# zha0ming1e/legged_mpc_control

Measured on AMD Instinct MI355X. Metric: QP solves/sec (Go1, horizon=10, 12 contacts); max GRF err vs exact-QP oracle, higher is better.
Workload: dtype f64; 1 GPU; go1_trot_h10_b1024; horizon=10, batch_per_gpu=1024, global_batch=1024, robot=go1, gait=trot, parallelism=dp1 (independent QP shards, no collective)

## Files before the change

legged_mpc_control_amd/build.py:

```python
from __future__ import annotations

import os
import shutil
import subprocess

PKG = os.path.dirname(os.path.abspath(__file__))
ROOT = os.path.dirname(PKG)
CSRC = os.path.join(PKG, "csrc")
LIBDIR = os.path.join(PKG, "lib")
LIB = os.path.join(LIBDIR, "liblmpc.so")
ARCH = "gfx950"
HIP_FLAGS = ["-mllvm", "-amdgpu-mfma-vgpr-form"]
KERNEL_FP = ["-ffp-contract=on", "-fno-signed-zeros"]
SCHED_FLAGS = {
    "lmpc_kernels.hip": ["-mllvm", "-amdgpu-sched-strategy=max-ilp"],
    "lmpc_dense.hip": ["-mllvm", "-amdgpu-sched-strategy=max-ilp"] + KERNEL_FP,
    "lmpc_lq.hip": ["-mllvm", "-amdgpu-sched-strategy=iterative-ilp"] + KERNEL_FP,
    "lmpc_fused.hip": ["-mllvm", "-amdgpu-sched-strategy=max-ilp"] + KERNEL_FP,
    "lmpc_gi.hip": ["-mllvm", "-amdgpu-sched-strategy=iterative-ilp"],
    "lmpc_hoqp.hip": ["-mllvm", "-amdgpu-sched-strategy=iterative-ilp"],
}

SOURCES = ["lmpc_kernels.hip", "lmpc_lq.hip", "lmpc_fused.hip", "lmpc_dense.hip", "lmpc_gi.hip", "lmpc_prep.hip", "lmpc_rollout.hip", "lmpc_hoqp.hip", "lmpc_wbc.hip", "lmpc_rbd.hip", "lmpc_sim.hip", "lmpc_contact.hip", "lmpc_stack.hip", "lmpc_est.hip", "lmpc_lowlevel.hip", "lmpc_capi.cpp",
           "hoqp_capi.cpp", "lmpc_host.cpp", "ConvexQPSolver.cpp"]
# ... 47 lines not shown
        os.path.join(ROOT, "include", "lmpc", "lmpc_rollout.h"), os.path.join(ROOT, "include", "lmpc", "lmpc_rbd.h"),
        os.path.join(ROOT, "include", "lmpc", "lmpc_sim.h"), os.path.join(ROOT, "include", "lmpc", "lmpc_stack.h"),
        os.path.join(ROOT, "include", "lmpc", "lmpc_est.h"), os.path.join(ROOT, "include", "lmpc", "lmpc_contact.h"),
        os.path.join(ROOT, "include", "lmpc", "lmpc_lowlevel.h"),
        os.path.join(ROOT, "include", "lmpc", "ConvexQPSolver.hpp"),
        os.path.abspath(__file__)]
    if not force and not _stale(LIB, deps):
        return LIB
    return _compile_lib(LIB, os.path.join(LIBDIR, "obj"), verbose=verbose)


MULTI_LIB = os.path.join(LIBDIR, "liblmpc_multi.so")


def build_multi(force: bool = False, verbose: bool = False) -> str:
    src = os.path.join(CSRC, "lmpc_multi.cpp")
    deps = [src, LIB, os.path.join(ROOT, "include", "lmpc", "lmpc_multi.h"), os.path.join(ROOT, "include", "lmpc", "lmpc.h"),
            os.path.abspath(__file__)]
    if not force and not _stale(MULTI_LIB, deps):
        return MULTI_LIB
    tmp = MULTI_LIB + ".tmp"
    cmd = [hipcc(), f"--offload-arch={ARCH}", "-O2", "-fPIC", "-shared", "-std=c++17", "-I", os.path.join(ROOT, "include"), "-o", tmp, src,
           "-L", LIBDIR, "-llmpc", "-Wl,-rpath,$ORIGIN", "-L/opt/rocm/lib", "-lrccl", "-Wl,-rpath,/opt/rocm/lib"]
    if verbose:
        print(" ".join(cmd))
    subprocess.run(cmd, check=True)
    os.replace(tmp, MULTI_LIB)
    return MULTI_LIB


def build_stamps(force: bool = False) -> str:
    srcs = [os.path.join(CSRC, s) for s in SOURCES]
    out = os.path.join(ROOT, "tools", "build", "liblmpc_stamps.so")
    if not force and not _stale(out, srcs + [os.path.join(CSRC, h) for h in HEADERS]):
        return out
    return _compile_lib(out, os.path.join(ROOT, "tools", "build", "obj_stamps"), defines=["LMPC_STAMPS"])


def build_variant(tag: str, defines, force: bool = False, flags=()) -> str:
    srcs = [os.path.join(CSRC, s) for s in SOURCES]
    out = os.path.join(ROOT, "tools", "build", f"liblmpc_{tag}.so")
    if not force and not _stale(out, srcs + [os.path.join(CSRC, h) for h in HEADERS]):
        return out
    return _compile_lib(out, os.path.join(ROOT, "tools", "build", f"obj_{tag}"), defines=defines, flags=flags)


TEST_BUILD = os.path.join(ROOT, "tests", "build")
TEST_VARIANTS = {
    "bugza": (["LMPC_BUG_ZA"], ("lmpc_lq.hip", "lmpc_fused.hip")),
    "bugza_nokkt": (["LMPC_BUG_ZA", "LMPC_KKT_OFF"], ("lmpc_lq.hip", "lmpc_fused.hip")),
    "bugyaw": (["LMPC_BUG_YAW"], ("lmpc_lq.hip", "lmpc_fused.hip")),
    "bugyaw_nokkt": (["LMPC_BUG_YAW", "LMPC_KKT_OFF"], ("lmpc_lq.hip", "lmpc_fused.hip")),
    "noschur": (["LMPC_POLISH_SCHUR=0"], ("lmpc_dense.hip", "lmpc_lq.hip", "lmpc_fused.hip")),
    "diag2tile": (["LMPC_DIAG_TWO_TILES"], ("lmpc_dense.hip", "lmpc_lq.hip", "lmpc_fused.hip")),
}


def build_test_variants(force: bool = False) -> dict:
    build_native()
    out = {}
    for tag, (defines, only) in TEST_VARIANTS.items():
        path = os.path.join(TEST_BUILD, f"liblmpc_{tag}.so")
        deps = [os.path.join(CSRC, s) for s in SOURCES] + [os.path.join(CSRC, h) for h in HEADERS] + [LIB]
        if force or _stale(path, deps):
            _compile_lib(path, os.path.join(TEST_BUILD, f"obj_{tag}"), defines=defines, only=only)
        out[tag] = path
    return out


def build_cpp_test(force: bool = False) -> str:
    src = os.path.join(ROOT, "tests", "cpp", "grf_update_test.cpp")
    out = os.path.join(ROOT, "tests", "cpp", "build", "grf_update_test")
    if not force and not _stale(out, [src, LIB]):
        return out
    os.makedirs(os.path.dirname(out), exist_ok=True)
    cmd = [hipcc(), "-O2", "-std=c++17", "-I", os.path.join(ROOT, "include"), "-o", out, src,
           "-L", LIBDIR, "-llmpc", f"-Wl,-rpath,{LIBDIR}"]
    subprocess.run(cmd, check=True)
    return out


def build_cpp_multi_test(force: bool = False) -> str:
    src = os.path.join(ROOT, "tests", "cpp", "multi_test.cpp")
    out = os.path.join(ROOT, "tests", "cpp", "build", "multi_test")
    if not force and not _stale(out, [src, LIB, MULTI_LIB]):
        return out
    os.makedirs(os.path.dirname(out), exist_ok=True)
    cmd = [hipcc(), "-O2", "-std=c++17", "-I", os.path.join(ROOT, "include"), "-o", out, src,
           "-L", LIBDIR, "-llmpc_multi", "-llmpc", f"-Wl,-rpath,{LIBDIR}"]
    subprocess.run(cmd, check=True)
    return out


def build_cpp_eigen_test(force: bool = False) -> str:
    src = os.path.join(ROOT, "tests", "cpp", "eigen_dropin_test.cpp")
    stub = os.path.join(ROOT, "tests", "cpp", "eigen_dropin")
    out = os.path.join(ROOT, "tests", "cpp", "build", "eigen_dropin_test")
    hdr = os.path.join(ROOT, "include", "lmpc", "ConvexQPSolverEigen.hpp")
    if not force and not _stale(out, [src, hdr, LIB]):
        return out
    os.makedirs(os.path.dirname(out), exist_ok=True)
    cmd = [hipcc(), "-O2", "-std=c++17", "-Wall", "-I", stub, "-I", os.path.join(ROOT, "include"), "-o", out, src,
           "-L", LIBDIR, "-llmpc", f"-Wl,-rpath,{LIBDIR}"]
    subprocess.run(cmd, check=True)
    return out

# ... 94 lines not shown
```

legged_mpc_control_amd/csrc/lmpc_dense.hip:

```cpp
#include <hip/hip_runtime.h>

#include <cmath>
#include <cstdint>

#include "lmpc/lmpc.h"
#include "lmpc_device.h"
#include "lmpc_kernel_common.h"
#include "lmpc_dense_common.h"

namespace lmpc {

#ifdef LMPC_STAMPS
constexpr int DSTAMP_N = 14;
__device__ unsigned long long lmpc_dense_stamps[4096][DSTAMP_N];
#define DSTAMP_DECL unsigned long long _ds_acc[DSTAMP_N] = {}; unsigned long long _ds_t0 = __builtin_readcyclecounter();
#define DSTAMP(i) do { const unsigned long long _t = __builtin_readcyclecounter(); _ds_acc[i] += _t - _ds_t0; _ds_t0 = _t; } while (0)
#define DSTAMP_FLUSH(qp) do { if (threadIdx.x == 0 && (qp) < 4096) for (int _i = 0; _i < DSTAMP_N; ++_i) lmpc_dense_stamps[qp][_i] = _ds_acc[_i]; } while (0)
#define DS_PARAMS , unsigned long long (&_ds_acc)[DSTAMP_N], unsigned long long& _ds_t0
#define DS_ARGS , _ds_acc, _ds_t0
#else
#define DS_PARAMS
#define DS_ARGS
#define DSTAMP_DECL
#define DSTAMP(i) do {} while (0)
#define DSTAMP_FLUSH(qp) do {} while (0)
#endif

#ifdef LMPC_KKT_DIAG
__device__ double lmpc_kkt_diag_dense[LMPC_KKT_DIAG_QPS][4];
extern "C" int lmpc_debug_kkt_dense(double* out, int nqp) {
    if (nqp > LMPC_KKT_DIAG_QPS) nqp = LMPC_KKT_DIAG_QPS;
    return hipMemcpyFromSymbol(out, HIP_SYMBOL(lmpc_kkt_diag_dense), (size_t)nqp * 4 * sizeof(double)) == hipSuccess
               ? nqp : -1;
}
extern "C" int lmpc_debug_kkt_dense_clear(void) {
    static double zeros[LMPC_KKT_DIAG_QPS * 4];
    return hipMemcpyToSymbol(HIP_SYMBOL(lmpc_kkt_diag_dense), zeros, sizeof(zeros)) == hipSuccess ? 0 : -1;
}
#endif

#ifdef LMPC_REFINE_DIAG
__device__ double lmpc_refine_diag[LMPC_KKT_DIAG_QPS][4];
extern "C" int lmpc_debug_refine(double* out, int nqp) {
    if (nqp > LMPC_KKT_DIAG_QPS) nqp = LMPC_KKT_DIAG_QPS;
    return hipMemcpyFromSymbol(out, HIP_SYMBOL(lmpc_refine_diag), (size_t)nqp * 4 * sizeof(double)) == hipSuccess
               ? nqp : -1;
}
extern "C" int lmpc_debug_refine_clear(void) {
    static double zeros[LMPC_KKT_DIAG_QPS * 4];
    return hipMemcpyToSymbol(HIP_SYMBOL(lmpc_refine_diag), zeros, sizeof(zeros)) == hipSuccess ? 0 : -1;
}
#endif

}

#include "lmpc_dense_kernel.h"

namespace lmpc {

template <bool TERRAIN>
__global__ void __launch_bounds__(64) lmpc_dense_kernel(const DevParams prm, const double* __restrict__ rec,
                                                        const uint8_t* __restrict__ contact,
                                                        const double* __restrict__ normals, int batch,
                                                        double* __restrict__ grf, int32_t* __restrict__ status,
                                                        int32_t* __restrict__ iters, uint8_t* __restrict__ done_out) {
    (void)dense_body<TERRAIN>(prm, rec, contact, normals, batch, grf, status, iters, done_out);
}

template __global__ void lmpc_dense_kernel<false>(const DevParams, const double*, const uint8_t*, const double*, int,
                                                  double*, int32_t*, int32_t*, uint8_t*);
template __global__ void lmpc_dense_kernel<true>(const DevParams, const double*, const uint8_t*, const double*, int,
                                                 double*, int32_t*, int32_t*, uint8_t*);

#ifdef LMPC_STAMPS
extern "C" int lmpc_debug_condense_stamps(unsigned long long* out, int nqp) {
    if (nqp > 4096) nqp = 4096;
    return hipMemcpyFromSymbol(out, HIP_SYMBOL(lmpc_condense_stamps), (size_t)nqp * 5 * sizeof(unsigned long long)) ==
                   hipSuccess ? nqp : -1;
}
extern "C" int lmpc_debug_dense_stamps(unsigned long long* out, int nqp) {
    if (nqp > 4096) nqp = 4096;
    return hipMemcpyFromSymbol(out, HIP_SYMBOL(lmpc_dense_stamps), (size_t)nqp * DSTAMP_N * sizeof(unsigned long long)) ==
                   hipSuccess ? nqp : -1;
}
#endif

size_t dense_lds_bytes(int H) {
    const int doubles = 40 + 72 + 24 + 36 + 10 * DN_TILE + 64 * 3 + 180 + 60 + 64 + 2 * H + 12 * H + 64 + DN_SCR_MIN;
    return (size_t)doubles * sizeof(double) + (20 + 33) * sizeof(int);
}

hipError_t launch_dense(const DevParams& prm, const double* rec, const uint8_t* contact, const double* normals,
                        int batch, double* grf, int32_t* status, int32_t* iters, uint8_t* done, hipStream_t stream) {
    const size_t lds = dense_lds_bytes(prm.H);
    const dim3 grid(batch), block(LMPC_WAVE);
    if (normals) {
        (void)hipFuncSetAttribute((const void*)lmpc_dense_kernel<true>, hipFuncAttributeMaxDynamicSharedMemorySize,
                                  (int)lds);
        hipLaunchKernelGGL(lmpc_dense_kernel<true>, grid, block, lds, stream, prm, rec, contact, normals, batch, grf,
                           status, iters, done);
    } else {
        (void)hipFuncSetAttribute((const void*)lmpc_dense_kernel<false>, hipFuncAttributeMaxDynamicSharedMemorySize,
                                  (int)lds);
// ... 8 lines not shown
```

legged_mpc_control_amd/csrc/lmpc_dense_common.h:

```cpp
#pragma once
#include <hip/hip_runtime.h>

#include <cmath>
#include <cstdint>

#include "lmpc/lmpc.h"
#include "lmpc_device.h"
#include "lmpc_kernel_common.h"

namespace lmpc {

constexpr int DN_TILE = 256;
size_t dense_lds_bytes(int H);

__device__ __forceinline__ constexpr int tix(int r, int c) { return r * 4 - r * (r - 1) / 2 + (c - r); }
__device__ __forceinline__ constexpr int uix(int a, int b) { return a == 0 ? b - 1 : a == 1 ? b + 1 : 5; }
__device__ __forceinline__ int toff(int r, int c) { return (r >> 2) * 64 + (r & 3) * 16 + c; }
__device__ __forceinline__ int vidx(int b, int a) { return 16 * (b / 5) + 3 * (b % 5) + a; }
__device__ __forceinline__ int sym3(int p, int q) {
    const int lo = p < q ? p : q, hi = p < q ? q : p;
    return lo == 0 ? hi : lo == 1 ? 2 + hi : 5;
}

__device__ __forceinline__ d4 tprod(const d4& X, const d4& Y, d4 acc) {
// ... 468 lines not shown
        out.uit[i] = W[i];
        out.ui[i] = tr[(4 * i + g) * 17 + c];
    }
    return out;
}


__device__ __forceinline__ unsigned tile_masks(int nls, unsigned coupled) {
    return __builtin_amdgcn_readfirstlane(((1u << nls) - 1u) & coupled);
}
__device__ __forceinline__ int tile_mask(unsigned masks, int t) { return (int)((masks >> (5 * t)) & 31u); }

__device__ __forceinline__ double h_matvec(const DSmem& S, const ldouble* x, ldouble* tmp, int lane) {
    const int lc = lane & 15, lr = lane >> 4;
    double xr[4][4], xc[4];
#pragma unroll
    for (int b = 0; b < 4; ++b) {
#pragma unroll
        for (int i = 0; i < 4; ++i) xr[b][i] = x[16 * b + 4 * i + lr];
        xc[b] = x[16 * b + lc];
    }
    double pc[4] = {0.0, 0.0, 0.0, 0.0};
    double pr[3][4] = {{0.0, 0.0, 0.0, 0.0}, {0.0, 0.0, 0.0, 0.0}, {0.0, 0.0, 0.0, 0.0}};
#pragma unroll
    for (int r = 0; r < 4; ++r) {
#pragma unroll
        for (int c = r; c < 4; ++c) {
            const int k = tix(r, c);
#pragma unroll
            for (int i = 0; i < 4; ++i) {
                const double h = S.Ht[k * DN_TILE + i * 64 + lane];
                pc[c] = fma(h, xr[r][i], pc[c]);
                if (c > r) pr[r][i] = fma(h, xc[c], pr[r][i]);
            }
        }
    }
#pragma unroll
    for (int r = 0; r < 3; ++r) {
        double rs[4];
        row_sum4(pr[r], rs);
        if (lc == 0) {
#pragma unroll
            for (int i = 0; i < 4; ++i) tmp[16 * r + 4 * i + lr] = rs[i];
        }
    }
    double yc[4];
#pragma unroll
    for (int c = 0; c < 4; ++c) yc[c] = group_sum4(pc[c]);
    LMPC_SYNC();
    const double ys = lr == 0 ? yc[0] : lr == 1 ? yc[1] : lr == 2 ? yc[2] : yc[3];
    return ys + (lr < 3 ? tmp[lane < 48 ? lane : 0] : 0.0);
}

struct DenseRec {
    double v[4];
};
static_assert(33 + 12 * DENSE_MAX_H <= 4 * 64, "DenseRec holds a whole record");
__device__ __forceinline__ DenseRec dense_rec_load(const double* __restrict__ rec, int qp, int H, int lane) {
    const int RL = 33 + 12 * H;
    const double* rin = rec + (size_t)qp * RL;
    DenseRec r;
#pragma unroll
    for (int q = 0; q < 4; ++q) {
        const int i = lane + 64 * q;
        r.v[q] = rin[i < RL ? i : 0];
    }
    return r;
}

template <bool TERRAIN>
__device__ __forceinline__ int dense_prologue(const DevParams& prm, const DSmem& S, const DenseRec& rv,
                                              const double* __restrict__ normals, int qp, int H,
                                              unsigned long long smask, bool stl, int lane) {
    const int RL = 33 + 12 * H;
    const double dt = prm.dt;
#pragma unroll
    for (int q = 0; q < 4; ++q) {
        const int i = lane + 64 * q;
        if (i < 33) S.hdr[i] = rv.v[q];
        else if (i < RL) S.xr[i - 33] = rv.v[q];
    }
    const int rank = __builtin_amdgcn_mbcnt_hi((unsigned)(smask >> 32), __builtin_amdgcn_mbcnt_lo((unsigned)smask, 0));
    if (stl) S.lsm[rank] = lane;
    if (lane <= H) {
        const unsigned long long below = (lane >= 16) ? smask : (smask & ((1ull << (4 * lane)) - 1ull));
        S.fb[lane] = __popcll(below);
    }
    if (TERRAIN && lane < 4) {
        const double* nin = normals + (size_t)qp * 12 + 3 * lane;
        const double n0 = nin[0], n1 = nin[1], n2 = nin[2];
        const double nn = sqrt(n0 * n0 + n1 * n1 + n2 * n2);
        const double nx = n0 / nn, ny = n1 / nn, c = n2 / nn;
        const double h = 1.0 / (1.0 + c);
        const double R[9] = {1.0 - nx * nx * h, -nx * ny * h, nx, -nx * ny * h, 1.0 - ny * ny * h, ny, -nx, -ny, c};
#pragma unroll
        for (int e = 0; e < 9; ++e) S.tf[9 * lane + e] = R[e];
    }
    LMPC_SYNC();
    double iw[9];
    {
        const ldouble* R = S.hdr + LMPC_REC_ROT;
        double RI[9], Iw[9];
        for (int i = 0; i < 3; ++i)
            for (int j = 0; j < 3; ++j)
                RI[i * 3 + j] = R[i * 3 + 0] * prm.Ib[0 * 3 + j] + R[i * 3 + 1] * prm.Ib[1 * 3 + j] + R[i * 3 + 2] * prm.Ib[2 * 3 + j];
        for (int i = 0; i < 3; ++i)
// ... 69 lines not shown
```

legged_mpc_control_amd/csrc/lmpc_dense_kernel.h:

```cpp
#pragma once
#include <hip/hip_runtime.h>

#include <cmath>
#include <cstdint>

#include "lmpc/lmpc.h"
#include "lmpc_device.h"
#include "lmpc_kernel_common.h"
#include "lmpc_dense_common.h"

#ifndef DSTAMP
#define DS_PARAMS
#define DS_ARGS
#define DSTAMP_DECL
#define DSTAMP(i) do {} while (0)
#define DSTAMP_FLUSH(qp) do {} while (0)
#endif

#ifndef LMPC_POLISH_SCHUR
#define LMPC_POLISH_SCHUR 1
#endif

namespace lmpc {

constexpr int LMPC_SCHUR_KMAX = 6;
constexpr int LMPC_SCHUR_SLOPE2 = 4;
constexpr int LMPC_SCHUR_LIM2 = 10;
constexpr double LMPC_DENSE_Z0 = 1.0;
#ifdef LMPC_REFINE_DIAG
constexpr double LMPC_REFINE_SR = 0.0;
#else
constexpr double LMPC_REFINE_SR = 1e-12;
#endif

static_assert(48 + 4 * LMPC_SCHUR_KMAX + 2 * LMPC_SCHUR_KMAX + LMPC_SCHUR_KMAX * LMPC_SCHUR_KMAX <= 120 &&
                  120 + LMPC_SCHUR_KMAX + 1 <= 128, "range-space scratch layout");
constexpr int DN_SCHUR_SV = 120;

template <typename P>
__device__ __forceinline__ int ncols3(const P* T) {
    int n = 0;
#pragma unroll
    for (int q = 0; q < 3; ++q) n += (T[q] != 0.0 || T[3 + q] != 0.0 || T[6 + q] != 0.0) ? 1 : 0;
    return n;
}
__device__ __forceinline__ int wave_count3(int k) {
    return __popcll(__ballot(k & 1)) + 2 * __popcll(__ballot(k & 2)) + 4 * __popcll(__ballot(k & 4));
}
__device__ __forceinline__ int wave_prefix3(int k, unsigned long long below) {
    return __popcll(__ballot(k & 1) & below) + 2 * __popcll(__ballot(k & 2) & below) +
           4 * __popcll(__ballot(k & 4) & below);
}

struct SchurLeg {
    int kc, kr;
    bool ok;
};
__device__ __forceinline__ SchurLeg schur_leg(bool chg, int act, int bact, bool nap, const ldouble* Tb,
                                              const double Tn[9], double mu, double fzmax) {
    SchurLeg r{0, 0, true};
    if (!chg) return r;
    const bool bap = (bact & 3) == 3 || (bact & 12) == 12;
    if (bap && nap) return r;
    const int cm = act & bact;
    double Tc[9], uc[3];
    (void)leg_basis(cm, mu, fzmax, Tc, uc);
    const int nb = ncols3(Tb), nc = ncols3(Tc), nn = ncols3(Tn);
    r.kc = nc - nb;
    r.kr = nap ? nc : __popc(act & ~bact);
    r.ok = r.kc >= 0 && r.kc <= 3 && r.kr <= 3 && (!bap || !(cm & 16)) && (!nap || !((act | bact) & 16)) &&
           (nap || nn == nc - r.kr);
    return r;
}

template <bool TERRAIN>
__device__ __forceinline__ bool dense_body(const DevParams prm, const double* __restrict__ rec,
                                           const uint8_t* __restrict__ contact, const double* __restrict__ normals,
                                           int batch, double* __restrict__ grf, int32_t* __restrict__ status,
                                           int32_t* __restrict__ iters, uint8_t* __restrict__ done_out) {
    extern __shared__ __attribute__((aligned(16))) double dn_smem[];
    const int qp = blockIdx.x;
    if (qp >= batch) return true;
    const int lane = threadIdx.x;
    const int H = prm.H;
    const uint8_t cbyte = contact[(size_t)qp * 4 * H + (lane < 4 * H ? lane : 0)];
    const DenseRec rv = dense_rec_load(rec, qp, H, lane);
    const bool stl = lane < 4 * H && cbyte != 0;
    const unsigned long long smask = __ballot(stl);
    const int nls = __popcll(smask);
    if (nls > DENSE_MAX_LS || nls == 0) return false;
    const DSmem S = dcarve(dn_smem, H);
    const double mu = prm.mu, fzmax = prm.fmax, dt = prm.dt;
    DSTAMP_DECL

    const int rank = dense_prologue<TERRAIN>(prm, S, rv, normals, qp, H, smask, stl, lane);
    DSTAMP(0);
    dense_condense<TERRAIN>(prm, S, H, nls, smask, lane);
    constexpr int NT = 4;
    DSTAMP(1);

    const bool st = lane < nls;
    int lk = 0, lj = 0;
    if (st) {
        const int id = S.lsm[lane];
        lk = id >> 2;
        lj = id & 3;
    }
    double f[3], s[5], z[5], is[5];
    {
        const double cnt = st ? (double)(S.fb[lk + 1] - S.fb[lk]) : 1.0;
        f[0] = f[1] = 0.0;
        f[2] = st ? fmin(0.5 * fzmax, prm.mass * prm.grav / cnt) : 0.0;
        double o[5];
        cons_resid(f, mu, fzmax, o);
#pragma unroll
        for (int i = 0; i < 5; ++i) {
            s[i] = st ? -o[i] : 1.0;
            is[i] = 1.0 / s[i];
            z[i] = LMPC_DENSE_Z0 * is[i];
        }
    }
    double u[3] = {0.0, 0.0, 0.0}, rt[3] = {0.0, 0.0, 0.0};
    int qstatus = LMPC_QP_CONVERGED, ipm_it = 0, prounds = 0;
    bool done = false;
    enum { PRED = 0, CORR = 1, POLISH = 2 };
    const double mc = 5.0 * nls, imc = 1.0 / mc;
    double tol = prm.tol_mu;
    int att = 0, rd = 0, it_end = min(prm.max_iter, prm.dense_polish_iter), mode = PRED, act = 0;
    int keep_tiles = 0;
    unsigned cmask = 0;
    bool apex = false;
    int bact = 0;
    bool have_base = false, schur = false;
    int nsch = 0, ncol = 0;
    double mu_c = 0.0, smu = 0.0, sz = 0.0;
    d4 Tl[10], Ui[4], UiT[4];
    const int lc = lane & 15, lr = lane >> 4;
    int lblk_reg = -1, lblk_q = 0, lblk_off = 0, ldg_reg = -1;
#pragma unroll
    for (int i = 0; i < 4; ++i) {
        const int r = lr + 4 * i;
        if (r < 15 && lc < 15 && r / 3 == lc / 3) {
            lblk_reg = i;
            lblk_q = r / 3;
            lblk_off = 3 * (r % 3) + lc % 3;
            if (r == lc) ldg_reg = i;
        }
    }
#if LMPC_POLISH_SCHUR
    auto schur_ksolve = [&](const double (&cv)[LMPC_SCHUR_KMAX], double (&sv)[LMPC_SCHUR_KMAX], double& kmin) -> bool {
        constexpr int KM = LMPC_SCHUR_KMAX;
        const ldouble* U = S.scr + 48;
        const ldouble* uleg = U + 4 * KM;
        const ldouble* utyp = uleg + KM;
        const ldouble* Cb = utyp + KM;
        const ldouble* Wc = S.scr + 128;
        double Am[KM][KM], sg[KM];
        int rb_[KM];
        bool rw[KM];
#pragma unroll
        for (int i = 0; i < KM; ++i) {
            const bool iv = i < nsch;
            rw[i] = iv && utyp[iv ? i : 0] < 0.5;
            rb_[i] = iv ? (int)uleg[i] : 0;
            sg[i] = rw[i] ? -1.0 : 1.0;
        }
#pragma unroll
        for (int i = 0; i < KM; ++i) {
            const bool iv = i < nsch;
#pragma unroll
            for (int j = 0; j <= i; ++j) {
                const bool jv = j < nsch;
                double v = (iv && jv) ? Cb[KM * i + j] : (i == j ? 1.0 : 0.0);
                if (iv && jv) {
                    if (rw[i]) {
#pragma unroll
                        for (int q = 0; q < 3; ++q) v = fma(-U[4 * i + q], Wc[64 * j + vidx(rb_[i], q)], v);
                    } else if (rw[j]) {
#pragma unroll
                        for (int q = 0; q < 3; ++q) v = fma(-U[4 * j + q], Wc[64 * i + vidx(rb_[j], q)], v);
                    }
                }
                Am[i][j] = v;
            }
        }
        bool bad = false;
        double dd[KM];
#pragma unroll
        for (int c = 0; c < KM; ++c) {
            double d = Am[c][c];
#pragma unroll
            for (int b = 0; b < c; ++b) d = fma(-Am[c][b], Am[c][b] * dd[b], d);
            bad |= !(sg[c] * d > 1e-14 * fabs(Am[c][c]));
            if (c < nsch) kmin = fmin(kmin, fabs(d) / fabs(Am[c][c]));
            dd[c] = d;
            const double inv = rcp_nr(d != 0.0 ? d : 1.0);
#pragma unroll
            for (int r = c + 1; r < KM; ++r) {
                double v = Am[r][c];
#pragma unroll
                for (int b = 0; b < c; ++b) v = fma(-Am[r][b], Am[c][b] * dd[b], v);
                Am[r][c] = v * inv;
            }
        }
#pragma unroll
        for (int r = 0; r < KM; ++r) {
            double v = cv[r];
#pragma unroll
            for (int b = 0; b < r; ++b) v = fma(-Am[r][b], sv[b], v);
            sv[r] = v;
        }
#pragma unroll
        for (int r = 0; r < KM; ++r) sv[r] = sv[r] * rcp_nr(dd[r] != 0.0 ? dd[r] : 1.0);
#pragma unroll
        for (int r = KM - 1; r >= 0; --r) {
            double v = sv[r];
#pragma unroll
            for (int b = r + 1; b < KM; ++b) v = fma(-Am[b][r], sv[b], v);
            sv[r] = v;
        }
        return bad;
    };
    bool force_fact = false, refact_done = false;
#endif
    for (;;) {
        if (mode == PRED) {
            if (ipm_it >= prm.dense_iter_cap) break;
            double loc = 0.0;
            if (st) {
#pragma unroll
                for (int i = 0; i < 5; ++i) loc += s[i] * z[i];
            }
            DSTAMP(2);
            sz = wave_sum(loc);
            mu_c = sz * imc;
            DSTAMP(12);
            if (mu_c < tol || ipm_it >= it_end) {
                act = 0;
                if (st) {
#pragma unroll
                    for (int i = 0; i < 5; ++i)
                        if (z[i] > LMPC_ACT_RATIO * s[i]) act |= 1 << i;
                    const double fm = fmax(fabs(f[0]), fmax(fabs(f[1]), fabs(f[2])));
                    if (fm < 1e-6 * fzmax) act = 15;
                }
                mode = POLISH;
                rd = 0;
                keep_tiles = 0;
                have_base = false;
            } else {
                double W[5] = {0, 0, 0, 0, 0}, wv[5] = {0, 0, 0, 0, 0};
                if (st) {
#pragma unroll
                    for (int i = 0; i < 5; ++i) {
                        W[i] = z[i] * is[i];
                        wv[i] = W[i] * (s[i] - (i == 4 ? fzmax : 0.0));
                    }
                }
                const double sx = W[0] + W[1], sy = W[2] + W[3];
                if (st) {
                    ldouble* bk = S.blk + 9 * lane;
                    const double dxz = mu * (W[0] - W[1]), dyz = mu * (W[2] - W[3]), dzz = mu * mu * (sx + sy) + W[4];
                    bk[0] = sx;  bk[1] = 0.0; bk[2] = dxz;
                    bk[3] = 0.0; bk[4] = sy;  bk[5] = dyz;
                    bk[6] = dxz; bk[7] = dyz; bk[8] = dzz;
                }
                cons_tw(wv, mu, rt);
            }
            DSTAMP(13);
        }
        double Tn[9], upn[3];
        if (mode == POLISH) {
            ++prounds;
            apex = false;
            double (&T)[9] = Tn;
            if (st) apex = leg_basis(act, mu, fzmax, T, upn);
            schur = false;
#if LMPC_POLISH_SCHUR
            if (have_base && !force_fact) {
                const SchurLeg sl = schur_leg(st && act != bact, act, bact, apex, S.blk + 9 * lane, T, mu, fzmax);
                const int k = sl.kc + sl.kr;
                nsch = wave_count3(k);
                ncol = wave_count3(sl.kc);
                const unsigned long long dif = __ballot(st && act != bact);
                const int kt = dif ? (__ffsll((long long)dif) - 1) / 5 : 4;
                schur = __all(sl.ok) && nsch + ncol <= LMPC_SCHUR_KMAX &&
                        2 * nsch + LMPC_SCHUR_SLOPE2 * kt <= LMPC_SCHUR_LIM2;
            }
            if (!schur) {
                const unsigned long long dif = __ballot(have_base && act != bact);
                keep_tiles = have_base && dif ? (__ffsll((long long)dif) - 1) / 5 : 0;
                force_fact = false;
            }
#endif
        }
        if (mode == POLISH && !schur) {
            S.vec2[lane] = 0.0;
            LMPC_SYNC();
            bool coupled = false;
            if (st) {
                const double (&T)[9] = Tn;
                const double (&up)[3] = upn;
#pragma unroll
                for (int p = 0; p < 3; ++p) S.lup[3 * lane + p] = up[p];
                ldouble* bk = S.blk + 9 * lane;
#pragma unroll
                for (int e = 0; e < 9; ++e) bk[e] = T[e];
#pragma unroll
                for (int e = 0; e < 9; ++e) coupled |= T[e] != 0.0;
#pragma unroll
                for (int p = 0; p < 3; ++p) S.vec2[vidx(lane, p)] = up[p];
            }
            cmask = (unsigned)__ballot(coupled);
        }
        if (schur) {
        } else if (mode != POLISH) {
            if (st) {
#pragma unroll
                for (int a = 0; a < 3; ++a) S.vec[vidx(lane, a)] = -(S.gv[vidx(lane, a)] + rt[a]);
            }
            LMPC_SYNC();
        } else {
            LMPC_SYNC();
            const double hv = h_matvec(S, S.vec2, S.scr, lane) + S.gv[lane];
            LMPC_SYNC();
            S.vec2[lane] = hv;
#if LMPC_POLISH_SCHUR
            S.lhg[lane] = hv;
#endif
            LMPC_SYNC();
            if (st) {
#pragma unroll
                for (int a = 0; a < 3; ++a) {
                    double v = 0.0;
#pragma unroll
                    for (int p = 0; p < 3; ++p) v += S.blk[9 * lane + p * 3 + a] * S.vec2[vidx(lane, p)];
                    S.vec[vidx(lane, a)] = -v;
                }
            }
// ... 96 lines not shown
                if (b > 0) {
                    double part = 0.0;
#pragma unroll
                    for (int a = 0; a < b; ++a) {
#pragma unroll
                        for (int i = 0; i < 4; ++i) part = fma(Tl[tix(a, b)][i], y[a][i], part);
                    }
                    acc -= group_sum4(part);
                }
                double pp[4], rs[4];
#pragma unroll
                for (int i = 0; i < 4; ++i) pp[i] = UiT[b][i] * acc;
                row_sum4(pp, rs);
#pragma unroll
                for (int i = 0; i < 4; ++i) y[b][i] = rs[i];
            }
            double xcol[4];
#pragma unroll
            for (int b = 3; b >= 0; --b) {
                if (b >= NT) continue;
                d4 acc = y[b];
                if (b + 1 < NT) {
                    double part[4] = {0.0, 0.0, 0.0, 0.0};
#pragma unroll
                    for (int c = b + 1; c < 4; ++c) {
                        if (c >= NT) continue;
#pragma unroll
                        for (int i = 0; i < 4; ++i) part[i] = fma(Tl[tix(b, c)][i], xcol[c], part[i]);
                    }
                    double rs[4];
                    row_sum4(part, rs);
#pragma unroll
                    for (int i = 0; i < 4; ++i) acc[i] -= rs[i];
                }
                double p = 0.0;
#pragma unroll
                for (int i = 0; i < 4; ++i) p = fma(UiT[b][i], acc[i], p);
                xcol[b] = group_sum4(p);
            }
            if (lr == 0) {
#pragma unroll
                for (int b = 0; b < 4; ++b) {
                    if (b >= NT) continue;
                    S.vec[16 * b + lc] = xcol[b];
                }
            }
            LMPC_SYNC();
        };
        double du[3] = {0.0, 0.0, 0.0};
        if (!schur) {
            solve_vec();
#if LMPC_POLISH_SCHUR
            if (mode == POLISH) {
                S.lua[lane] = S.vec[lane];
                bact = act;
                have_base = true;
            }
#endif
        }
#if LMPC_POLISH_SCHUR
        else {
            constexpr int KM = LMPC_SCHUR_KMAX;
            ldouble* U = S.scr + 48;
            ldouble* uleg = U + 4 * KM;
            ldouble* utyp = uleg + KM;
            ldouble* Cb = utyp + KM;
            ldouble* Wc = S.scr + 128;
            ldouble* Vc = Wc + 64 * nsch;
            const SchurLeg sl = schur_leg(st && act != bact, act, bact, apex, S.blk + 9 * lane, Tn, mu, fzmax);
            const unsigned long long below = (1ull << lane) - 1ull;
            const int e0 = wave_prefix3(sl.kc + sl.kr, below), c0 = wave_prefix3(sl.kc, below);
            if (lane < KM * KM) Cb[lane] = 0.0;
            LMPC_SYNC();
            if (sl.kc + sl.kr) {
                const ldouble* Tb = S.blk + 9 * lane;
                const ldouble* ub = S.lup + 3 * lane;
                double Tc[9], uc[3];
                (void)leg_basis(act & bact, mu, fzmax, Tc, uc);
                double tv[3][3];
                const int nb = ncols3(Tb);
                if (nb == 0) {
#pragma unroll
                    for (int j = 0; j < 3; ++j)
#pragma unroll
                        for (int p = 0; p < 3; ++p) tv[j][p] = Tc[3 * p + j];
                } else {
                    double best = -1.0, rb[3] = {0.0, 0.0, 0.0};
#pragma unroll
                    for (int q = 0; q < 3; ++q) {
                        double r[3] = {Tc[q], Tc[3 + q], Tc[6 + q]};
#pragma unroll
                        for (int m = 0; m < 2; ++m) {
                            const double pr = Tb[m] * r[0] + Tb[3 + m] * r[1] + Tb[6 + m] * r[2];
#pragma unroll
                            for (int p = 0; p < 3; ++p) r[p] = fma(-pr, Tb[3 * p + m], r[p]);
                        }
                        const double n2 = r[0] * r[0] + r[1] * r[1] + r[2] * r[2];
                        if (n2 > best) {
                            best = n2;
                            rb[0] = r[0]; rb[1] = r[1]; rb[2] = r[2];
                        }
                    }
                    const double in = rsq_nr(best > 0.0 ? best : 1.0);
#pragma unroll
                    for (int p = 0; p < 3; ++p) tv[0][p] = rb[p] * in;
                    const double b0 = Tb[0], b1 = Tb[3], b2 = Tb[6];
                    tv[1][0] = b1 * tv[0][2] - b2 * tv[0][1];
                    tv[1][1] = b2 * tv[0][0] - b0 * tv[0][2];
                    tv[1][2] = b0 * tv[0][1] - b1 * tv[0][0];
                    tv[2][0] = tv[2][1] = tv[2][2] = 0.0;
                }
                double rv[3][3], rbv[3];
                if (apex) {
#pragma unroll
                    for (int j = 0; j < 3; ++j) {
#pragma unroll
                        for (int p = 0; p < 3; ++p) rv[j][p] = Tc[3 * p + j];
                        rbv[j] = 0.0;
                    }
                } else {
                    const ActiveRows ar = active_rows(act & ~bact);
                    cons_rowvec(ar.i0, mu, rv[0]);
                    cons_rowvec(ar.i1, mu, rv[1]);
                    cons_rowvec(ar.i2, mu, rv[2]);
                    rbv[0] = ar.i0 == 4 ? fzmax : 0.0;
                    rbv[1] = ar.i1 == 4 ? fzmax : 0.0;
                    rbv[2] = ar.i2 == 4 ? fzmax : 0.0;
                }
#pragma unroll
                for (int j = 0; j < 3; ++j) {
                    if (j >= sl.kc) continue;
                    const int e = e0 + j;
                    double c = 0.0;
#pragma unroll
                    for (int p = 0; p < 3; ++p) {
                        U[4 * e + p] = tv[j][p];
                        c = fma(-tv[j][p], S.lhg[vidx(lane, p)], c);
                    }
                    U[4 * e + 3] = c;
                    uleg[e] = (double)lane;
                    utyp[e] = (double)(1 + c0 + j);
                }
#pragma unroll
                for (int i = 0; i < 3; ++i) {
                    if (i >= sl.kr) continue;
                    const int e = e0 + sl.kc + i;
#pragma unroll
                    for (int q = 0; q < 3; ++q)
                        U[4 * e + q] = fma(rv[i][0], Tb[q], fma(rv[i][1], Tb[3 + q], rv[i][2] * Tb[6 + q]));
                    U[4 * e + 3] = rbv[i] - fma(rv[i][0], ub[0], fma(rv[i][1], ub[1], rv[i][2] * ub[2]));
                    uleg[e] = (double)lane;
                    utyp[e] = 0.0;
#pragma unroll
                    for (int j = 0; j < 3; ++j) {
                        if (j >= sl.kc) continue;
                        const double a = rv[i][0] * tv[j][0] + rv[i][1] * tv[j][1] + rv[i][2] * tv[j][2];
                        Cb[KM * e + e0 + j] = a;
                        Cb[KM * (e0 + j) + e] = a;
                    }
                }
            }
            LMPC_SYNC();
            if (ncol) {
                const int w16 = lane & 15, bl = 5 * (lane >> 4) + w16 / 3, al = w16 % 3;
                const bool vl = w16 < 15 && bl < nls;
                for (int e = 0; e < nsch; ++e) {
                    const double ty = utyp[e];
                    if (ty < 0.5) continue;
                    const int be = (int)uleg[e];
                    S.vec2[lane] = 0.0;
                    LMPC_SYNC();
                    if (lane < 3) S.vec2[vidx(be, lane)] = U[4 * e + lane];
                    LMPC_SYNC();
                    const double h = h_matvec(S, S.vec2, S.scr, lane);
                    LMPC_SYNC();
                    S.vec2[lane] = h;
                    LMPC_SYNC();
                    double v = 0.0;
                    if (vl) {
#pragma unroll
                        for (int p = 0; p < 3; ++p) v = fma(S.blk[9 * bl + 3 * p + al], S.vec2[vidx(bl, p)], v);
                    }
                    Vc[64 * ((int)ty - 1) + lane] = v;
                    if (lane < nsch && utyp[lane] > 0.5) {
                        const int bj = (int)uleg[lane];
                        double c = 0.0;
#pragma unroll
                        for (int p = 0; p < 3; ++p) c = fma(U[4 * lane + p], S.vec2[vidx(bj, p)], c);
                        Cb[KM * lane + e] = c;
                    }
                    LMPC_SYNC();
                }
            }
            for (int e = 0; e < nsch; ++e) {
                const double ty = utyp[e];
                if (ty > 0.5) {
                    S.vec[lane] = Vc[64 * ((int)ty - 1) + lane];
                } else {
                    S.vec[lane] = 0.0;
                    LMPC_SYNC();
                    if (lane < 3) S.vec[vidx((int)uleg[e], lane)] = U[4 * e + lane];
                }
                LMPC_SYNC();
                solve_vec();
                Wc[64 * e + lane] = S.vec[lane];
            }
            LMPC_SYNC();
            if (ncol) {
                const double y0l = S.lua[lane];
                for (int e = 0; e < nsch; ++e) {
                    const double ty = utyp[e];
                    if (ty < 0.5) continue;
                    const double vl = Vc[64 * ((int)ty - 1) + lane];
                    const double cy = wave_sum(vl * y0l);
                    if (lane == 0) U[4 * e + 3] -= cy;
                    for (int f = e; f < nsch; ++f) {
                        if (utyp[f] < 0.5) continue;
                        const double g = wave_sum(vl * Wc[64 * f + lane]);
                        if (lane == 0) {
                            Cb[KM * e + f] -= g;
                            if (f != e) Cb[KM * f + e] -= g;
                        }
                    }
                }
                LMPC_SYNC();
            }
            double cv[KM], sv[KM];
#pragma unroll
            for (int i = 0; i < KM; ++i) {
                const bool iv = i < nsch;
                const bool rwi = iv && utyp[iv ? i : 0] < 0.5;
                const int rbi = iv ? (int)uleg[i] : 0;
                double c = iv ? U[4 * i + 3] : 0.0;
                if (rwi) {
#pragma unroll
                    for (int q = 0; q < 3; ++q) c = fma(-U[4 * i + q], S.lua[vidx(rbi, q)], c);
                }
                cv[i] = c;
            }
            double kmin = 1.0;
            const bool bad = schur_ksolve(cv, sv, kmin);
            double yv = S.lua[lane];
#pragma unroll
            for (int j = 0; j < KM; ++j)
                if (j < nsch) yv = fma(-Wc[64 * j + lane], sv[j], yv);
            if (ncol && !bad && st) {
#pragma unroll
                for (int j = 0; j < KM; ++j) {
                    if (j >= nsch || utyp[j] < 0.5 || (int)uleg[j] != lane) continue;
#pragma unroll
                    for (int p = 0; p < 3; ++p) du[p] = fma(U[4 * j + p], sv[j], du[p]);
                }
            }
            if (lane == 0) {
#pragma unroll
                for (int j = 0; j < KM; ++j) S.scr[DN_SCHUR_SV + j] = sv[j];
                S.scr[DN_SCHUR_SV + KM] = kmin;
            }
            S.vec[lane] = bad ? S.lua[lane] : yv;
            if (bad) have_base = false;
            LMPC_SYNC();
        }
#endif
        DSTAMP(5);
        u[0] = u[1] = u[2] = 0.0;
        if (st) {
            double y3[3];
#pragma unroll
            for (int a = 0; a < 3; ++a) y3[a] = S.vec[vidx(lane, a)];
            if (mode == POLISH) {
                const ldouble* Tb = S.blk + 9 * lane;
#pragma unroll
                for (int p = 0; p < 3; ++p)
                    u[p] = apex ? 0.0
                                : S.lup[3 * lane + p] + Tb[p * 3] * y3[0] + Tb[p * 3 + 1] * y3[1] + Tb[p * 3 + 2] * y3[2] +
                                      du[p];
            } else {
#pragma unroll
                for (int p = 0; p < 3; ++p) u[p] = y3[p];
            }
        }
        if (mode == PRED) {
            double amax = 1.0;
            double dsa[5], dza[5];
#pragma unroll
            for (int i = 0; i < 5; ++i) dsa[i] = dza[i] = 0.0;
            if (st) {
#pragma unroll
                for (int m = 0; m < 3; ++m) S.lua[3 * lane + m] = u[m];
            }
            if (st) {
                double o[5];
                cons_resid(u, mu, fzmax, o);
#pragma unroll
                for (int i = 0; i < 5; ++i) {
                    dsa[i] = -o[i] - s[i];
                    dza[i] = -z[i] - z[i] * is[i] * dsa[i];
                    if (dsa[i] < 0.0) amax = fmin(amax, -s[i] * __builtin_amdgcn_rcp(dsa[i]));
                    if (dza[i] < 0.0) amax = fmin(amax, -z[i] * __builtin_amdgcn_rcp(dza[i]));
                }
            }
            const double aa = wave_min(amax);
            double loc = 0.0;
            if (st) {
#pragma unroll
                for (int i = 0; i < 5; ++i) loc += (s[i] + aa * dsa[i]) * (z[i] + aa * dza[i]);
            }
            const double ratio = wave_sum(loc) / sz;
            smu = ratio * ratio * ratio * mu_c;
            if (st) {
                double wv[5];
#pragma unroll
                for (int i = 0; i < 5; ++i)
                    wv[i] = (z[i] * (s[i] - (i == 4 ? fzmax : 0.0)) + smu - dsa[i] * dza[i]) * is[i];
// ... 214 lines not shown
#pragma unroll
                            for (int i = 0; i < 5; ++i)
                                if (!((act >> i) & 1) && o[i] > prm.tol_p * fzmax) ok = false;
                            if (apex) {
                                ok = ok && !(g2[2] / mu < fabs(g2[0]) + fabs(g2[1]) - prm.tol_d * gs2);
                            } else {
                                const LegKkt kk = leg_kkt(act, g2, mu, -prm.tol_d * gs2);
                                ok = ok && kk.drop < 0 && kk.res <= prm.tol_d * gs2;
                            }
                        }
#ifdef LMPC_REFINE_DIAG
                        {
                            double dl = 0.0;
#pragma unroll
                            for (int p = 0; p < 3; ++p) dl = fmax(dl, fabs(ur[p] - u[p]));
                            dl = wave_max(dl);
                            const bool allok = __all(ok);
                            if (lane == 0 && qp < LMPC_KKT_DIAG_QPS) {
                                lmpc_refine_diag[qp][0] = sr / gscale;
                                lmpc_refine_diag[qp][1] = S.scr[DN_SCHUR_SV + KM];
                                lmpc_refine_diag[qp][2] = dl;
                                lmpc_refine_diag[qp][3] = allok ? 1.0 : 2.0;
                            }
                        }
#endif
                        if (__all(ok)) {
#pragma unroll
                            for (int p = 0; p < 3; ++p) u[p] = ur[p];
                        }
                    }
#endif
                    done = true;
                    break;
                }
#if LMPC_POLISH_SCHUR
                if (schur && !refact_done) {
                    force_fact = true;
                    refact_done = true;
                } else
#endif
                    rd = prm.max_rounds - 1;
            }
            keep_tiles = chg ? (__ffsll((long long)chg) - 1) / 5 : 0;
            if (++rd >= prm.max_rounds) {
                keep_tiles = 0;
                schur = false;
                if (++att >= prm.max_attempts) break;
                tol = retry_tol(tol, att);
                it_end += prm.max_iter;
                mode = PRED;
            }
        }
    }
    if (!done) {
        qstatus = LMPC_QP_MAX_ITER;
#pragma unroll
        for (int m = 0; m < 3; ++m) u[m] = f[m];
    }
    const int bad = st && (u[0] != u[0] || u[1] != u[1] || u[2] != u[2]);
    const bool anybad = __any(bad);
    if (done_out) {
        const bool keep = done && !anybad;
        if (lane == 0) done_out[qp] = keep ? 1 : 0;
        if (!keep) {
            DSTAMP_FLUSH(qp);
            return false;
        }
    }
    LMPC_SYNC();
    if (st) {
        double fo[3] = {u[0], u[1], u[2]};
        if constexpr (TERRAIN) {
            const ldouble* Rj = S.tf + 9 * lj;
#pragma unroll
            for (int p = 0; p < 3; ++p) fo[p] = Rj[3 * p] * u[0] + Rj[3 * p + 1] * u[1] + Rj[3 * p + 2] * u[2];
        }
#pragma unroll
        for (int p = 0; p < 3; ++p) S.vec[3 * lane + p] = fo[p];
    }
    LMPC_SYNC();
    double* gout = grf + (size_t)qp * 12 * H;
    if (lane < 4 * H) {
#pragma unroll
        for (int p = 0; p < 3; ++p) gout[3 * lane + p] = (anybad || !stl) ? 0.0 : S.vec[3 * (stl ? rank : 0) + p];
    }
    if (lane == 0) {
        if (status) status[qp] = anybad ? LMPC_QP_NAN : qstatus;
        if (iters) iters[qp] = ipm_it | (prounds << 16);
    }
    DSTAMP(2);
    DSTAMP_FLUSH(qp);
    return true;
}

}
```

legged_mpc_control_amd/csrc/lmpc_fused.hip:

```cpp
#include <hip/hip_runtime.h>

#include <algorithm>
#include <cstdint>

#include "lmpc/lmpc.h"
#include "lmpc_device.h"
#include "lmpc_kernel_common.h"

#if !defined(LMPC_STAMPS) && !defined(LMPC_KKT_DIAG) && !defined(LMPC_BUG_ZA) && !defined(LMPC_BUG_YAW) && \
    !defined(LMPC_KKT_OFF) && !defined(LMPC_LQ_DEBUG) && !defined(LMPC_REFINE_DIAG)
#define LMPC_FUSED 1
#include "lmpc_dense_kernel.h"
#include "lmpc_lq_kernel.h"
#else
#define LMPC_FUSED 0
#endif

namespace lmpc {

#if LMPC_FUSED
template <bool TERRAIN>
__global__ void __launch_bounds__(64, 1) lmpc_dense_lq_kernel(const DevParams prm, const double* __restrict__ rec,
                                                              const uint8_t* __restrict__ contact,
                                                              const double* __restrict__ normals, int batch,
                                                              double* __restrict__ grf, int32_t* __restrict__ status,
                                                              int32_t* __restrict__ iters, uint8_t* __restrict__ done) {
    if (!dense_body<TERRAIN>(prm, rec, contact, normals, batch, grf, status, iters, done))
        lq_body<1, TERRAIN, 1>(prm, rec, contact, normals, batch, grf, status, iters, done, true);
}
template __global__ void lmpc_dense_lq_kernel<false>(const DevParams, const double*, const uint8_t*, const double*,
                                                     int, double*, int32_t*, int32_t*, uint8_t*);
template __global__ void lmpc_dense_lq_kernel<true>(const DevParams, const double*, const uint8_t*, const double*,
                                                    int, double*, int32_t*, int32_t*, uint8_t*);
#endif

hipError_t launch_dense_lq(const DevParams& prm, const double* rec, const uint8_t* contact, const double* normals,
                           int batch, double* grf, int32_t* status, int32_t* iters, uint8_t* done, hipStream_t stream) {
#if LMPC_FUSED
    if (4 * prm.H > 64 || batch > 4 * prm.cus) return hipErrorNotSupported;
    const size_t lds = std::max(dense_lds_bytes(prm.H), lq_lds_bytes(prm.H));
    const dim3 grid(batch), block(LMPC_WAVE);
    if (normals) {
        (void)hipFuncSetAttribute((const void*)lmpc_dense_lq_kernel<true>, hipFuncAttributeMaxDynamicSharedMemorySize,
                                  (int)lds);
        hipLaunchKernelGGL(lmpc_dense_lq_kernel<true>, grid, block, lds, stream, prm, rec, contact, normals, batch, grf,
                           status, iters, done);
    } else {
        (void)hipFuncSetAttribute((const void*)lmpc_dense_lq_kernel<false>, hipFuncAttributeMaxDynamicSharedMemorySize,
                                  (int)lds);
        hipLaunchKernelGGL(lmpc_dense_lq_kernel<false>, grid, block, lds, stream, prm, rec, contact, normals, batch, grf,
                           status, iters, done);
    }
    return hipGetLastError();
#else
    (void)prm, (void)rec, (void)contact, (void)normals, (void)batch, (void)grf, (void)status, (void)iters, (void)done;
    (void)stream;
    return hipErrorNotSupported;
#endif
}

}
```

Baseline: 7.003 million QP/s.

## Specialize Schur polish solve by size and replace basis-derived counts with bitmask

The Schur-complement polish solve is instantiated per active size (1..6) via a switch, so the small LDL factorization and solves run at the exact size instead of a masked KMAX=6 loop. Per-leg free-column counts now come from a popcount on the active mask rather than building leg bases, and the Schur leg data is computed once and reused. The column-by-Hessian product for Schur updates reads three Hessian tile entries directly instead of doing a full matvec with several syncs. The Schur acceptance thresholds are retuned and a debug diagnostic variant is added. Together this trims per-round polish work, at the cost of more code size and register pressure from six instantiations.

After: 7.374 million QP/s (median of 6 runs). 1.05x the previous value.

```diff
diff --git a/legged_mpc_control_amd/build.py b/legged_mpc_control_amd/build.py
--- a/legged_mpc_control_amd/build.py
+++ b/legged_mpc_control_amd/build.py
@@ -123,6 +123,7 @@
     "bugyaw": (["LMPC_BUG_YAW"], ("lmpc_lq.hip", "lmpc_fused.hip")),
     "bugyaw_nokkt": (["LMPC_BUG_YAW", "LMPC_KKT_OFF"], ("lmpc_lq.hip", "lmpc_fused.hip")),
     "noschur": (["LMPC_POLISH_SCHUR=0"], ("lmpc_dense.hip", "lmpc_lq.hip", "lmpc_fused.hip")),
+    "schurdiag": (["LMPC_SCHUR_DIAG"], ("lmpc_dense.hip", "lmpc_lq.hip", "lmpc_fused.hip")),
     "diag2tile": (["LMPC_DIAG_TWO_TILES"], ("lmpc_dense.hip", "lmpc_lq.hip", "lmpc_fused.hip")),
 }
 
diff --git a/legged_mpc_control_amd/csrc/lmpc_dense.hip b/legged_mpc_control_amd/csrc/lmpc_dense.hip
--- a/legged_mpc_control_amd/csrc/lmpc_dense.hip
+++ b/legged_mpc_control_amd/csrc/lmpc_dense.hip
@@ -11,7 +11,7 @@
 namespace lmpc {
 
 #ifdef LMPC_STAMPS
-constexpr int DSTAMP_N = 14;
+constexpr int DSTAMP_N = 15;
 __device__ unsigned long long lmpc_dense_stamps[4096][DSTAMP_N];
 #define DSTAMP_DECL unsigned long long _ds_acc[DSTAMP_N] = {}; unsigned long long _ds_t0 = __builtin_readcyclecounter();
 #define DSTAMP(i) do { const unsigned long long _t = __builtin_readcyclecounter(); _ds_acc[i] += _t - _ds_t0; _ds_t0 = _t; } while (0)
@@ -49,6 +49,20 @@
 extern "C" int lmpc_debug_refine_clear(void) {
     static double zeros[LMPC_KKT_DIAG_QPS * 4];
     return hipMemcpyToSymbol(HIP_SYMBOL(lmpc_refine_diag), zeros, sizeof(zeros)) == hipSuccess ? 0 : -1;
+}
+#endif
+
+#ifdef LMPC_SCHUR_DIAG
+constexpr int LMPC_SCHUR_DIAG_QPS = 4096;
+__device__ double lmpc_schur_diag[LMPC_SCHUR_DIAG_QPS][6];
+extern "C" int lmpc_debug_schur(double* out, int nqp) {
+    if (nqp > LMPC_SCHUR_DIAG_QPS) nqp = LMPC_SCHUR_DIAG_QPS;
+    return hipMemcpyFromSymbol(out, HIP_SYMBOL(lmpc_schur_diag), (size_t)nqp * 6 * sizeof(double)) == hipSuccess
+               ? nqp : -1;
+}
+extern "C" int lmpc_debug_schur_clear(void) {
+    static double zeros[LMPC_SCHUR_DIAG_QPS * 6];
+    return hipMemcpyToSymbol(HIP_SYMBOL(lmpc_schur_diag), zeros, sizeof(zeros)) == hipSuccess ? 0 : -1;
 }
 #endif
 
diff --git a/legged_mpc_control_amd/csrc/lmpc_dense_common.h b/legged_mpc_control_amd/csrc/lmpc_dense_common.h
--- a/legged_mpc_control_amd/csrc/lmpc_dense_common.h
+++ b/legged_mpc_control_amd/csrc/lmpc_dense_common.h
@@ -544,6 +544,17 @@
     return ys + (lr < 3 ? tmp[lane < 48 ? lane : 0] : 0.0);
 }
 
+__device__ __forceinline__ double h_col3(const DSmem& S, int b, const double (&e3)[3], int lane) {
+    const int tv = lane >> 4, vw = lane & 15;
+    const int tw = b / 5, sw = 3 * (b - 5 * tw);
+    const bool up = tv <= tw;
+    const ldouble* T = S.Ht + (up ? tix(tv, tw) : tix(tw, tv)) * DN_TILE;
+    double h = 0.0;
+#pragma unroll
+    for (int q = 0; q < 3; ++q) h = fma(T[up ? toff(vw, sw + q) : toff(sw + q, vw)], e3[q], h);
+    return h;
+}
+
 struct DenseRec {
     double v[4];
 };
diff --git a/legged_mpc_control_amd/csrc/lmpc_dense_kernel.h b/legged_mpc_control_amd/csrc/lmpc_dense_kernel.h
--- a/legged_mpc_control_amd/csrc/lmpc_dense_kernel.h
+++ b/legged_mpc_control_amd/csrc/lmpc_dense_kernel.h
@@ -3,6 +3,7 @@
 
 #include <cmath>
 #include <cstdint>
+#include <type_traits>
 
 #include "lmpc/lmpc.h"
 #include "lmpc_device.h"
@@ -24,8 +25,8 @@
 namespace lmpc {
 
 constexpr int LMPC_SCHUR_KMAX = 6;
-constexpr int LMPC_SCHUR_SLOPE2 = 4;
-constexpr int LMPC_SCHUR_LIM2 = 10;
+constexpr int LMPC_SCHUR_SLOPE2 = 3;
+constexpr int LMPC_SCHUR_LIM2 = 11;
 constexpr double LMPC_DENSE_Z0 = 1.0;
 #ifdef LMPC_REFINE_DIAG
 constexpr double LMPC_REFINE_SR = 0.0;
@@ -56,16 +57,14 @@
     int kc, kr;
     bool ok;
 };
-__device__ __forceinline__ SchurLeg schur_leg(bool chg, int act, int bact, bool nap, const ldouble* Tb,
-                                              const double Tn[9], double mu, double fzmax) {
+__device__ __forceinline__ int leg_free(int a) { return ((a & 3) == 3 || (a & 12) == 12) ? 0 : 3 - __popc(a & 31); }
+__device__ __forceinline__ SchurLeg schur_leg(bool chg, int act, int bact, bool nap) {
     SchurLeg r{0, 0, true};
     if (!chg) return r;
     const bool bap = (bact & 3) == 3 || (bact & 12) == 12;
     if (bap && nap) return r;
     const int cm = act & bact;
-    double Tc[9], uc[3];
-    (void)leg_basis(cm, mu, fzmax, Tc, uc);
-    const int nb = ncols3(Tb), nc = ncols3(Tc), nn = ncols3(Tn);
+    const int nb = leg_free(bact), nc = leg_free(cm), nn = leg_free(act);
     r.kc = nc - nb;
     r.kr = nap ? nc : __popc(act & ~bact);
     r.ok = r.kc >= 0 && r.kc <= 3 && r.kr <= 3 && (!bap || !(cm & 16)) && (!nap || !((act | bact) & 16)) &&
@@ -148,55 +147,52 @@
         }
     }
 #if LMPC_POLISH_SCHUR
-    auto schur_ksolve = [&](const double (&cv)[LMPC_SCHUR_KMAX], double (&sv)[LMPC_SCHUR_KMAX], double& kmin) -> bool {
+    auto schur_ksolve_n = [&](auto nc, const double (&cv)[LMPC_SCHUR_KMAX], double (&sv)[LMPC_SCHUR_KMAX],
+                              double& kmin) -> bool {
         constexpr int KM = LMPC_SCHUR_KMAX;
+        constexpr int N = decltype(nc)::value;
         const ldouble* U = S.scr + 48;
         const ldouble* uleg = U + 4 * KM;
         const ldouble* utyp = uleg + KM;
         const ldouble* Cb = utyp + KM;
         const ldouble* Wc = S.scr + 128;
-        double Am[KM][KM], sg[KM];
-        int rb_[KM];
-        bool rw[KM];
-#pragma unroll
-        for (int i = 0; i < KM; ++i) {
-            const bool iv = i < nsch;
-            rw[i] = iv && utyp[iv ? i : 0] < 0.5;
-            rb_[i] = iv ? (int)uleg[i] : 0;
+        double Am[N][N], sg[N];
+        int rb_[N];
+        bool rw[N];
+#pragma unroll
+        for (int i = 0; i < N; ++i) {
+            rw[i] = utyp[i] < 0.5;
+            rb_[i] = (int)uleg[i];
             sg[i] = rw[i] ? -1.0 : 1.0;
         }
 #pragma unroll
-        for (int i = 0; i < KM; ++i) {
-            const bool iv = i < nsch;
+        for (int i = 0; i < N; ++i) {
 #pragma unroll
             for (int j = 0; j <= i; ++j) {
-                const bool jv = j < nsch;
-                double v = (iv && jv) ? Cb[KM * i + j] : (i == j ? 1.0 : 0.0);
-                if (iv && jv) {
-                    if (rw[i]) {
-#pragma unroll
-                        for (int q = 0; q < 3; ++q) v = fma(-U[4 * i + q], Wc[64 * j + vidx(rb_[i], q)], v);
-                    } else if (rw[j]) {
-#pragma unroll
-                        for (int q = 0; q < 3; ++q) v = fma(-U[4 * j + q], Wc[64 * i + vidx(rb_[j], q)], v);
-                    }
+                double v = Cb[KM * i + j];
+                if (rw[i]) {
+#pragma unroll
+                    for (int q = 0; q < 3; ++q) v = fma(-U[4 * i + q], Wc[64 * j + vidx(rb_[i], q)], v);
+                } else if (rw[j]) {
+#pragma unroll
+                    for (int q = 0; q < 3; ++q) v = fma(-U[4 * j + q], Wc[64 * i + vidx(rb_[j], q)], v);
                 }
                 Am[i][j] = v;
             }
         }
         bool bad = false;
-        double dd[KM];
-#pragma unroll
-        for (int c = 0; c < KM; ++c) {
+        double dd[N];
+#pragma unroll
+        for (int c = 0; c < N; ++c) {
             double d = Am[c][c];
 #pragma unroll
             for (int b = 0; b < c; ++b) d = fma(-Am[c][b], Am[c][b] * dd[b], d);
             bad |= !(sg[c] * d > 1e-14 * fabs(Am[c][c]));
-            if (c < nsch) kmin = fmin(kmin, fabs(d) / fabs(Am[c][c]));
+            kmin = fmin(kmin, fabs(d) / fabs(Am[c][c]));
             dd[c] = d;
             const double inv = rcp_nr(d != 0.0 ? d : 1.0);
 #pragma unroll
-            for (int r = c + 1; r < KM; ++r) {
+            for (int r = c + 1; r < N; ++r) {
                 double v = Am[r][c];
 #pragma unroll
                 for (int b = 0; b < c; ++b) v = fma(-Am[r][b], Am[c][b] * dd[b], v);
@@ -204,24 +200,40 @@
             }
         }
 #pragma unroll
-        for (int r = 0; r < KM; ++r) {
+        for (int r = 0; r < KM; ++r) sv[r] = 0.0;
+#pragma unroll
+        for (int r = 0; r < N; ++r) {
             double v = cv[r];
 #pragma unroll
             for (int b = 0; b < r; ++b) v = fma(-Am[r][b], sv[b], v);
             sv[r] = v;
         }
 #pragma unroll
-        for (int r = 0; r < KM; ++r) sv[r] = sv[r] * rcp_nr(dd[r] != 0.0 ? dd[r] : 1.0);
-#pragma unroll
-        for (int r = KM - 1; r >= 0; --r) {
+        for (int r = 0; r < N; ++r) sv[r] = sv[r] * rcp_nr(dd[r] != 0.0 ? dd[r] : 1.0);
+#pragma unroll
+        for (int r = N - 1; r >= 0; --r) {
             double v = sv[r];
 #pragma unroll
-            for (int b = r + 1; b < KM; ++b) v = fma(-Am[b][r], sv[b], v);
+            for (int b = r + 1; b < N; ++b) v = fma(-Am[b][r], sv[b], v);
             sv[r] = v;
         }
         return bad;
     };
+    auto schur_ksolve = [&](const double (&cv)[LMPC_SCHUR_KMAX], double (&sv)[LMPC_SCHUR_KMAX], double& kmin) -> bool {
+        static_assert(LMPC_SCHUR_KMAX == 6, "one instance per size");
+        switch (nsch) {
+            case 1: return schur_ksolve_n(std::integral_constant<int, 1>{}, cv, sv, kmin);
+            case 2: return schur_ksolve_n(std::integral_constant<int, 2>{}, cv, sv, kmin);
+            case 3: return schur_ksolve_n(std::integral_constant<int, 3>{}, cv, sv, kmin);
+            case 4: return schur_ksolve_n(std::integral_constant<int, 4>{}, cv, sv, kmin);
+            case 5: return schur_ksolve_n(std::integral_constant<int, 5>{}, cv, sv, kmin);
+            default: return schur_ksolve_n(std::integral_constant<int, 6>{}, cv, sv, kmin);
+        }
+    };
     bool force_fact = false, refact_done = false;
+#ifdef LMPC_SCHUR_DIAG
+    int sd_rounds = 0, sd_ent = 0, sd_col = 0, sd_max = 0, sd_run = 0, sd_runmax = 0, sd_mis = 0;
+#endif
 #endif
     for (;;) {
         if (mode == PRED) {
@@ -270,6 +282,7 @@
             DSTAMP(13);
         }
         double Tn[9], upn[3];
+        SchurLeg sl{0, 0, true};
         if (mode == POLISH) {
             ++prounds;
             apex = false;
@@ -278,13 +291,13 @@
             schur = false;
 #if LMPC_POLISH_SCHUR
             if (have_base && !force_fact) {
-                const SchurLeg sl = schur_leg(st && act != bact, act, bact, apex, S.blk + 9 * lane, T, mu, fzmax);
+                sl = schur_leg(st && act != bact, act, bact, apex);
                 const int k = sl.kc + sl.kr;
                 nsch = wave_count3(k);
                 ncol = wave_count3(sl.kc);
                 const unsigned long long dif = __ballot(st && act != bact);
                 const int kt = dif ? (__ffsll((long long)dif) - 1) / 5 : 4;
-                schur = __all(sl.ok) && nsch + ncol <= LMPC_SCHUR_KMAX &&
+                schur = __all(sl.ok) && nsch > 0 && nsch + ncol <= LMPC_SCHUR_KMAX &&
                         2 * nsch + LMPC_SCHUR_SLOPE2 * kt <= LMPC_SCHUR_LIM2;
             }
             if (!schur) {
@@ -487,6 +500,9 @@
             solve_vec();
 #if LMPC_POLISH_SCHUR
             if (mode == POLISH) {
+#ifdef LMPC_SCHUR_DIAG
+                sd_run = 0;
+#endif
                 S.lua[lane] = S.vec[lane];
                 bact = act;
                 have_base = true;
@@ -502,11 +518,27 @@
             ldouble* Cb = utyp + KM;
             ldouble* Wc = S.scr + 128;
             ldouble* Vc = Wc + 64 * nsch;
-            const SchurLeg sl = schur_leg(st && act != bact, act, bact, apex, S.blk + 9 * lane, Tn, mu, fzmax);
             const unsigned long long below = (1ull << lane) - 1ull;
             const int e0 = wave_prefix3(sl.kc + sl.kr, below), c0 = wave_prefix3(sl.kc, below);
             if (lane < KM * KM) Cb[lane] = 0.0;
             LMPC_SYNC();
+#ifdef LMPC_SCHUR_DIAG
+            {
+                ++sd_rounds;
+                sd_ent += nsch;
+                sd_col += ncol;
+                sd_max = max(sd_max, nsch);
+                sd_runmax = max(sd_runmax, ++sd_run);
+                bool mis = false;
+                if (st && act != bact) {
+                    double Tk[9], uk[3];
+                    (void)leg_basis(act & bact, mu, fzmax, Tk, uk);
+                    mis = ncols3(S.blk + 9 * lane) != leg_free(bact) || ncols3(Tn) != leg_free(act) ||
+                          ncols3(Tk) != leg_free(act & bact);
+                }
+                sd_mis += __popcll(__ballot(mis));
+            }
+#endif
             if (sl.kc + sl.kr) {
                 const ldouble* Tb = S.blk + 9 * lane;
                 const ldouble* ub = S.lup + 3 * lane;
@@ -602,14 +634,8 @@
                 for (int e = 0; e < nsch; ++e) {
                     const double ty = utyp[e];
                     if (ty < 0.5) continue;
-                    const int be = (int)uleg[e];
-                    S.vec2[lane] = 0.0;
-                    LMPC_SYNC();
-                    if (lane < 3) S.vec2[vidx(be, lane)] = U[4 * e + lane];
-                    LMPC_SYNC();
-                    const double h = h_matvec(S, S.vec2, S.scr, lane);
-                    LMPC_SYNC();
-                    S.vec2[lane] = h;
+                    const double t3[3] = {U[4 * e], U[4 * e + 1], U[4 * e + 2]};
+                    S.vec2[lane] = h_col3(S, (int)uleg[e], t3, lane);
                     LMPC_SYNC();
                     double v = 0.0;
                     if (vl) {
@@ -695,6 +721,7 @@
             S.vec[lane] = bad ? S.lua[lane] : yv;
             if (bad) have_base = false;
             LMPC_SYNC();
+            DSTAMP(14);
         }
 #endif
         DSTAMP(5);
@@ -1015,6 +1042,13 @@
             }
         }
     }
+#if LMPC_POLISH_SCHUR && defined(LMPC_SCHUR_DIAG)
+    if (lane == 0 && qp < LMPC_SCHUR_DIAG_QPS) {
+        const int sd[6] = {sd_rounds, sd_ent, sd_col, sd_max, sd_runmax, sd_mis};
+#pragma unroll
+        for (int i = 0; i < 6; ++i) lmpc_schur_diag[qp][i] = (double)sd[i];
+    }
+#endif
     if (!done) {
         qstatus = LMPC_QP_MAX_ITER;
 #pragma unroll
diff --git a/legged_mpc_control_amd/csrc/lmpc_fused.hip b/legged_mpc_control_amd/csrc/lmpc_fused.hip
--- a/legged_mpc_control_amd/csrc/lmpc_fused.hip
+++ b/legged_mpc_control_amd/csrc/lmpc_fused.hip
@@ -8,7 +8,7 @@
 #include "lmpc_kernel_common.h"
 
 #if !defined(LMPC_STAMPS) && !defined(LMPC_KKT_DIAG) && !defined(LMPC_BUG_ZA) && !defined(LMPC_BUG_YAW) && \
-    !defined(LMPC_KKT_OFF) && !defined(LMPC_LQ_DEBUG) && !defined(LMPC_REFINE_DIAG)
+    !defined(LMPC_KKT_OFF) && !defined(LMPC_LQ_DEBUG) && !defined(LMPC_REFINE_DIAG) && !defined(LMPC_SCHUR_DIAG)
 #define LMPC_FUSED 1
 #include "lmpc_dense_kernel.h"
 #include "lmpc_lq_kernel.h"
```
